# PathologyFoundation/plip

Measured on NVIDIA H100. Metric: image-text pairs/sec (224x224, 77-tok), higher is better.
Workload: dtype bf16

## Files before the change

### plip_b200/csrc/gemm_wgmma.cu

```cuda
#include "gemm.cuh"
#include "wgmma.cuh"

#include <stdio.h>
#include <stdlib.h>

namespace plip {

namespace {

constexpr int BM = 64;
constexpr int BK = 64;
constexpr int kThreads = 288;
constexpr int kConsumerWarps = 8;
constexpr uint32_t A_STAGE = BM * BK * 2;
constexpr uint32_t kStoreStageBytes = 16 * 128;

constexpr int x_boxes(int BN, int EPI) {
  return EPI != EPI_BIAS_RESID_F32 ? 2 : BN == 192 ? 3 : 2;
}

template <int BN, int EPI>
struct Cfg {
  static constexpr uint32_t B_STAGE = BN * BK * 2;
  static constexpr uint32_t STAGE = A_STAGE + B_STAGE;
  static constexpr int XBOXES = x_boxes(BN, EPI);
  static constexpr uint32_t EPI_BYTES = kConsumerWarps * XBOXES * kStoreStageBytes;
  static constexpr uint32_t BAR_BYTES = EPI == EPI_BIAS_RESID_F32 ? 512 : 256;
  static constexpr uint32_t ALIGN_SLACK = 1024;
  static constexpr int kMaxStages = (227 * 1024 - BAR_BYTES - EPI_BYTES - ALIGN_SLACK) / STAGE;
  static constexpr int STAGES = kMaxStages > 8 ? 8 : kMaxStages;
  static constexpr uint32_t SMEM_BYTES = STAGES * STAGE + EPI_BYTES + BAR_BYTES + ALIGN_SLACK;
};

struct GemmDev {
  int M, N, K;
  const float* bias;
  const float* rowscale;
  void* out;
  int ldo;
  const float* pos;
  int patches, seq;
  const float* colsum;
  const float2* stats_in;
  int n_partials;
  __nv_bfloat16* xb_out;
  float2* stats_out;
};

template <bool F16, int BN>
__device__ __forceinline__ void wgmma_ss(float (&d)[BN / 2], uint64_t adesc, uint64_t bdesc, uint32_t scale_d) {
  if constexpr (BN == 128) wgmma_ss_n128<F16>(d, adesc, bdesc, scale_d);
  else if constexpr (BN == 192) wgmma_ss_n192<F16>(d, adesc, bdesc, scale_d);
  else wgmma_ss_n256<F16>(d, adesc, bdesc, scale_d);
}

__device__ __forceinline__ float2 ln_row_terms(const GemmDev& p, int grow) {
  float s1 = 0.f, s2 = 0.f;
#pragma unroll
  for (int j = 0; j < kStatSlots; ++j) {
    const float2 t = (grow < p.M && j < p.n_partials) ? __ldg(p.stats_in + static_cast<size_t>(grow) * kStatSlots + j)
                                                      : make_float2(0.f, 0.f);
    s1 += t.x;
    s2 += t.y;
  }
  const float inv_k = 1.0f / static_cast<float>(p.K);
  const float mean = s1 * inv_k;
  const float rstd = rsqrtf(fmaxf(s2 * inv_k - mean * mean, 0.f) + kLnEps);
  return make_float2(-rstd * mean, rstd);
}

template <int BN, int EPI, bool F16>
__device__ __forceinline__ void epilogue_warp(const GemmDev& p, const CUtensorMap* tmC, float (&d)[BN / 2], uint32_t stage_smem,
                                              uint32_t& stage_sel, uint32_t xbar, int row_base, int col_base, int n_blk, int lane,
                                              float2 ln0, float2 ln1) {
  constexpr bool LN_FOLD = (EPI == EPI_LN_BIAS_BF16 || EPI == EPI_LN_BIAS_GELU_BF16);
  constexpr bool GELU = (EPI == EPI_BIAS_GELU_BF16 || EPI == EPI_LN_BIAS_GELU_BF16);
  constexpr bool HAS_BIAS = (EPI == EPI_BIAS_BF16 || EPI == EPI_BIAS_GELU_BF16 || EPI == EPI_BIAS_RESID_F32 || LN_FOLD);
  constexpr bool OUT_BF16 = (EPI == EPI_BIAS_BF16 || EPI == EPI_BIAS_GELU_BF16 || LN_FOLD);
  const int q = lane & 3, rr = lane >> 2;
  const int row0 = row_base + rr, row1 = row0 + 8;

  if constexpr (EPI == EPI_NULL) {
    float acc = 0.f;
#pragma unroll
    for (int i = 0; i < BN / 2; ++i) acc += d[i];
    if (acc == 1.2345e30f && p.M < 0) reinterpret_cast<float*>(p.out)[0] = acc;
  } else if constexpr (OUT_BF16) {
#pragma unroll
    for (int blk = 0; blk < BN / 64; ++blk) {
      const uint32_t buf = stage_smem + (stage_sel & 1u) * kStoreStageBytes;
      ++stage_sel;
      if (lane == 0) tma_store_wait_read_but_one();
      __syncwarp();
#pragma unroll
      for (int jj = 0; jj < 8; ++jj) {
        const int j = blk * 8 + jj;
        const int col = col_base + 8 * j + 2 * q;
        const float2 b = __ldg(reinterpret_cast<const float2*>(p.bias + col));
        float v00 = d[4 * j + 0], v01 = d[4 * j + 1], v10 = d[4 * j + 2], v11 = d[4 * j + 3];
        if constexpr (LN_FOLD) {
          const float2 cs = __ldg(reinterpret_cast<const float2*>(p.colsum + col));
          v00 = fmaf(ln0.y, v00, fmaf(ln0.x, cs.x, b.x));
          v01 = fmaf(ln0.y, v01, fmaf(ln0.x, cs.y, b.y));
          v10 = fmaf(ln1.y, v10, fmaf(ln1.x, cs.x, b.x));
          v11 = fmaf(ln1.y, v11, fmaf(ln1.x, cs.y, b.y));
        } else {
          v00 += b.x; v01 += b.y; v10 += b.x; v11 += b.y;
        }
        if constexpr (GELU) {
          v00 = quick_gelu(v00); v01 = quick_gelu(v01); v10 = quick_gelu(v10); v11 = quick_gelu(v11);
        }
        st_shared_b32(buf + rr * 128 + ((jj ^ rr) << 4) + q * 4, pack_op2<F16>(v00, v01));
        st_shared_b32(buf + (rr + 8) * 128 + ((jj ^ rr) << 4) + q * 4, pack_op2<F16>(v10, v11));
      }
      fence_proxy_async_smem();
      __syncwarp();
      if (lane == 0) {
        tma_store_2d(tmC, buf, col_base + blk * 64, row_base);
        tma_store_commit();
      }
    }
  } else if constexpr (EPI == EPI_BIAS_RESID_F32) {
    constexpr int kChunkCols = 32;
    constexpr int kChunks = BN / kChunkCols;
    constexpr int NB = x_boxes(BN, EPI);
    static_assert(kChunks % NB == 0, "every tile must start at staging block 0");
    constexpr int kUses = kChunks / NB;
    const bool ok0 = row0 < p.M, ok1 = row1 < p.M;
    const bool emit = p.xb_out != nullptr;
    const size_t o0 = static_cast<size_t>(ok0 ? row0 : 0) * p.ldo + col_base + 2 * q;
    const size_t o1 = o0 + 8 * static_cast<size_t>(p.ldo);
    uint32_t ph0 = 0;
    if constexpr (kUses % 2 != 0) ph0 = stage_sel++ & 1u;
    auto fetch = [&](int c) {
      if (lane == 0) {
        const uint32_t bar = xbar + 8u * (c % NB);
        mbar_arrive_expect_tx(bar, kStoreStageBytes);
        tma_load_2d(stage_smem + (c % NB) * kStoreStageBytes, tmC, bar, 2 * (col_base + c * kChunkCols), row_base);
      }
    };
    if (lane == 0) tma_store_wait_read();
    __syncwarp();
#pragma unroll
    for (int c = 0; c < NB; ++c) fetch(c);
    float st[2][2] = {};
#pragma unroll
    for (int c = 0; c < kChunks; ++c) {
      const int h = c < kChunks / 2 ? 0 : 1;
      mbar_wait(xbar + 8u * (c % NB), ph0 ^ ((c / NB) & 1u));
      const uint32_t buf = stage_smem + (c % NB) * kStoreStageBytes;
#pragma unroll
      for (int jj = 0; jj < kChunkCols / 8; ++jj) {
        const int j = c * (kChunkCols / 8) + jj;
        const int col = col_base + 8 * j + 2 * q;
        const uint32_t xoff = (((2 * jj + (q >> 1)) ^ rr) << 4) + (q & 1) * 8;
        const float2 b = __ldg(reinterpret_cast<const float2*>(p.bias + col));
        const float2 v0 = make_float2(d[4 * j + 0] + b.x, d[4 * j + 1] + b.y);
        const float2 v1 = make_float2(d[4 * j + 2] + b.x, d[4 * j + 3] + b.y);
        if (ok0) {
          const float2 x = ld_shared_f32x2(buf + rr * 128 + xoff);
          const float2 y = make_float2(x.x + v0.x, x.y + v0.y);
          st_shared_f32x2(buf + rr * 128 + xoff, y);
          if (emit) {
            *reinterpret_cast<uint32_t*>(p.xb_out + o0 + 8 * j) = pack_op2<F16>(y.x, y.y);
            st[0][0] += y.x + y.y;
            st[0][1] = fmaf(y.x, y.x, fmaf(y.y, y.y, st[0][1]));
          }
        }
        if (ok1) {
          const float2 x = ld_shared_f32x2(buf + (rr + 8) * 128 + xoff);
          const float2 y = make_float2(x.x + v1.x, x.y + v1.y);
          st_shared_f32x2(buf + (rr + 8) * 128 + xoff, y);
          if (emit) {
            *reinterpret_cast<uint32_t*>(p.xb_out + o1 + 8 * j) = pack_op2<F16>(y.x, y.y);
            st[1][0] += y.x + y.y;
            st[1][1] = fmaf(y.x, y.x, fmaf(y.y, y.y, st[1][1]));
          }
        }
      }
      fence_proxy_async_smem();
      __syncwarp();
      if (lane == 0) {
        tma_store_2d(tmC, buf, 2 * (col_base + c * kChunkCols), row_base);
        tma_store_commit();
      }
      if (c + NB < kChunks) {
        if (lane == 0) tma_store_wait_read();
        fetch(c + NB);
      }
      if (emit && (c + 1) % (kChunks / 2) == 0) {
#pragma unroll
        for (int r = 0; r < 2; ++r) {
          float a = st[r][0], b = st[r][1];
#pragma unroll
          for (int o = 1; o < 4; o <<= 1) {
            a += __shfl_xor_sync(0xffffffffu, a, o);
            b += __shfl_xor_sync(0xffffffffu, b, o);
          }
          if (q == 0 && (r == 0 ? ok0 : ok1))
            p.stats_out[static_cast<size_t>(row0 + 8 * r) * kStatSlots + 2 * n_blk + h] = make_float2(a, b);
          st[r][0] = 0.f;
          st[r][1] = 0.f;
        }
      }
    }
  } else {
    float* out = reinterpret_cast<float*>(p.out);
    const bool ok0 = row0 < p.M, ok1 = row1 < p.M;
    float rs0 = 1.f, rs1 = 1.f;
    size_t o0 = static_cast<size_t>(ok0 ? row0 : 0) * p.ldo, o1 = static_cast<size_t>(ok1 ? row1 : 0) * p.ldo;
    if constexpr (EPI == EPI_SIM_F32) {
      rs0 = ok0 ? __ldg(p.rowscale + row0) : 0.f;
      rs1 = ok1 ? __ldg(p.rowscale + row1) : 0.f;
    }
    size_t q0 = 0, q1 = 0;
    if constexpr (EPI == EPI_PATCH_F32) {
      const int r0 = ok0 ? row0 : 0, r1 = ok1 ? row1 : 0;
      const int b0 = r0 / p.patches, b1 = r1 / p.patches;
      o0 = static_cast<size_t>(b0 * p.seq + 1 + (r0 - b0 * p.patches)) * p.ldo;
      o1 = static_cast<size_t>(b1 * p.seq + 1 + (r1 - b1 * p.patches)) * p.ldo;
      q0 = static_cast<size_t>(1 + (r0 - b0 * p.patches)) * p.N;
      q1 = static_cast<size_t>(1 + (r1 - b1 * p.patches)) * p.N;
    }
#pragma unroll
    for (int j = 0; j < BN / 8; ++j) {
      const int col = col_base + 8 * j + 2 * q;
      float2 v0 = make_float2(d[4 * j + 0], d[4 * j + 1]), v1 = make_float2(d[4 * j + 2], d[4 * j + 3]);
      if constexpr (HAS_BIAS) {
        const float2 b = __ldg(reinterpret_cast<const float2*>(p.bias + col));
        v0.x += b.x; v0.y += b.y; v1.x += b.x; v1.y += b.y;
      }
      if constexpr (EPI == EPI_SIM_F32) {
        const float2 cs = __ldg(reinterpret_cast<const float2*>(p.bias + col));
        if (ok0) *reinterpret_cast<float2*>(out + o0 + col) = make_float2(v0.x * rs0 * cs.x, v0.y * rs0 * cs.y);
        if (ok1) *reinterpret_cast<float2*>(out + o1 + col) = make_float2(v1.x * rs1 * cs.x, v1.y * rs1 * cs.y);
      } else if constexpr (EPI == EPI_PATCH_F32) {
        if (ok0) {
          const float2 e = __ldg(reinterpret_cast<const float2*>(p.pos + q0 + col));
          *reinterpret_cast<float2*>(out + o0 + col) = make_float2(v0.x + e.x, v0.y + e.y);
        }
        if (ok1) {
          const float2 e = __ldg(reinterpret_cast<const float2*>(p.pos + q1 + col));
          *reinterpret_cast<float2*>(out + o1 + col) = make_float2(v1.x + e.x, v1.y + e.y);
        }
      } else {
        if (ok0) *reinterpret_cast<float2*>(out + o0 + col) = v0;
        if (ok1) *reinterpret_cast<float2*>(out + o1 + col) = v1;
      }
    }
  }
}

template <int CG, int BN, int EPI, bool F16>
__global__ void __launch_bounds__(kThreads, 1)
gemm_kernel(const __grid_constant__ CUtensorMap tmA, const __grid_constant__ CUtensorMap tmB,
            const __grid_constant__ CUtensorMap tmC, const GemmDev p) {
  using C = Cfg<BN, EPI>;
  constexpr int STAGES = C::STAGES;
  extern __shared__ uint8_t smem_raw[];
  const uint32_t smem_base = (smem_u32(smem_raw) + 1023u) & ~1023u;
  const uint32_t epi_base = smem_base + STAGES * C::STAGE;
  const uint32_t bar_base = epi_base + C::EPI_BYTES;
  auto full_bar = [&](int s) { return bar_base + 8u * s; };
  auto empty_bar = [&](int s) { return bar_base + 8u * (STAGES + s); };
  const uint32_t resid_bar = bar_base + 8u * (2 * STAGES);
  static_assert(8 * (2 * STAGES + (EPI == EPI_BIAS_RESID_F32 ? C::XBOXES * kConsumerWarps : 0)) <= C::BAR_BYTES,
                "barrier area too small");

  const int warp = threadIdx.x >> 5;
  const int lane = threadIdx.x & 31;
  const int wg = warp >> 2;
  const uint32_t cta_rank = (CG > 1) ? cluster_ctarank() : 0u;

  if (threadIdx.x == 0) {
    tma_prefetch_desc(&tmA);
    tma_prefetch_desc(&tmB);
    for (int s = 0; s < STAGES; ++s) {
      mbar_init(full_bar(s), 1);
      mbar_init(empty_bar(s), CG);
    }
    if constexpr (EPI == EPI_BIAS_RESID_F32) {
      tma_prefetch_desc(&tmC);
      for (int i = 0; i < C::XBOXES * kConsumerWarps; ++i) mbar_init(resid_bar + 8u * i, 1);
    }
    fence_mbar_init();
  }
  if constexpr (CG > 1) cluster_sync_all(); else __syncthreads();

  const int num_n_blk = p.N / BN;
  const int num_m_blk = (p.M + BM * CG - 1) / (BM * CG);
  const int num_tiles = num_m_blk * num_n_blk;
  const int num_kb = p.K / BK;
  const int tile0 = blockIdx.x / CG;
  const int tile_step = gridDim.x / CG;
  const int my_tiles = (num_tiles - tile0 + tile_step - 1) / tile_step;

  if (wg == 2) {
    if (lane == 0) {
      int s = 0;
      uint32_t ph = 0;
      for (int t = tile0; t < num_tiles; t += tile_step) {
        const int m0 = ((t / num_n_blk) * CG + cta_rank) * BM;
        const int n0 = (t % num_n_blk) * BN;
        for (int kb = 0; kb < num_kb; ++kb) {
          mbar_wait(empty_bar(s), ph ^ 1u);
          const uint32_t sa = smem_base + s * C::STAGE;
          const uint32_t sb = sa + A_STAGE;
          mbar_arrive_expect_tx(full_bar(s), C::STAGE);
          tma_load_2d(sa, &tmA, full_bar(s), kb * BK, m0);
          if constexpr (CG == 1) {
            tma_load_2d(sb, &tmB, full_bar(s), kb * BK, n0);
          } else {
            tma_load_2d_mc(sb + cta_rank * (C::B_STAGE / 2), &tmB, full_bar(s), kb * BK, n0 + cta_rank * (BN / 2), 0x3);
          }
          if (++s == STAGES) { s = 0; ph ^= 1u; }
        }
      }
    }
    __syncwarp();
  } else {
    const int wtid = threadIdx.x & 127;
    auto release = [&](int s) {
      if (wtid == 0) mbar_arrive(empty_bar(s));
      if constexpr (CG > 1) {
        if (wtid == 32) mbar_arrive_cluster(mapa_shared(empty_bar(s), cta_rank ^ 1u));
      }
    };
    float d[BN / 2];
    int s = 0;
    uint32_t ph = 0;
    auto skip_tile = [&]() {
      s += num_kb;
      ph ^= static_cast<uint32_t>(s / STAGES) & 1u;
      s %= STAGES;
    };
    uint32_t stage_sel = 0;
    const uint32_t my_turn = 1u + wg, other_turn = 2u - wg;
    const int rounds = (my_tiles + 1) / 2;
    if (wg == 1) skip_tile();
    for (int r = 0; r < rounds; ++r) {
      const int i = 2 * r + wg;
      const int t = tile0 + i * tile_step;
      const int n_blk = t % num_n_blk;
      const int m0 = ((t / num_n_blk) * CG + cta_rank) * BM;
      const int wrow = m0 + (warp & 3) * 16;
      float2 ln0 = make_float2(0.f, 1.f), ln1 = make_float2(0.f, 1.f);
      if constexpr (EPI == EPI_LN_BIAS_BF16 || EPI == EPI_LN_BIAS_GELU_BF16) {
        if (i < my_tiles) {
          ln0 = ln_row_terms(p, wrow + (lane >> 2));
          ln1 = ln_row_terms(p, wrow + (lane >> 2) + 8);
        }
      }
      if (wg == 1 || r > 0) named_barrier_sync<256>(my_turn);
      if (i >= my_tiles) break;
      int prev = -1;
      for (int kb = 0; kb < num_kb; ++kb) {
        mbar_wait(full_bar(s), ph);
        const uint32_t sa = smem_base + s * C::STAGE;
        const uint64_t adesc = make_smem_desc_sw128(sa, 1024, 16);
        const uint64_t bdesc = make_smem_desc_sw128(sa + A_STAGE, 1024, 16);
        wgmma_pin(d);
        wgmma_fence();
#pragma unroll
        for (int k = 0; k < BK / 16; ++k) wgmma_ss<F16, BN>(d, adesc + 2 * k, bdesc + 2 * k, (kb | k) != 0 ? 1u : 0u);
        wgmma_commit();
        wgmma_wait<1>();
        if (prev >= 0) release(prev);
        prev = s;
        if (++s == STAGES) { s = 0; ph ^= 1u; }
      }
      if (wg == 0 || r + 1 < rounds) named_barrier_arrive<256>(other_turn);
      wgmma_wait<0>();
      wgmma_pin(d);
      release(prev);
      skip_tile();
      epilogue_warp<BN, EPI, F16>(p, &tmC, d, epi_base + warp * C::XBOXES * kStoreStageBytes, stage_sel,
                                  resid_bar + 8u * C::XBOXES * warp, wrow,
                                  n_blk * BN, n_blk, lane, ln0, ln1);
    }
    if (lane == 0) tma_store_wait_all();
    __syncwarp();
  }
  if constexpr (CG > 1) cluster_sync_all();
}

int env_int(const char* name, int dflt) {
  const char* v = getenv(name);
  return v ? atoi(v) : dflt;
}

template <int CG, int BN, int EPI, bool F16>
int launch_inst(const GemmArgs& g, cudaStream_t stream) {
  using C = Cfg<BN, EPI>;
  auto kern = gemm_kernel<CG, BN, EPI, F16>;
  static unsigned long long configured = 0;
  static int max_groups = 0;
  if (first_use_on_device(configured)) {
    PLIP_CUDA_CHECK(cudaFuncSetAttribute(kern, cudaFuncAttributeMaxDynamicSharedMemorySize, (int)C::SMEM_BYTES));
    int dev = 0, sms = 0;
    PLIP_CUDA_CHECK(cudaGetDevice(&dev));
    PLIP_CUDA_CHECK(cudaDeviceGetAttribute(&sms, cudaDevAttrMultiProcessorCount, dev));
    max_groups = sms / CG;
    if (CG >= 2) {
      cudaLaunchConfig_t q = {};
      q.gridDim = dim3(sms / CG * CG);
      q.blockDim = dim3(kThreads);
      q.dynamicSmemBytes = C::SMEM_BYTES;
      cudaLaunchAttribute qa[1];
      qa[0].id = cudaLaunchAttributeClusterDimension;
      qa[0].val.clusterDim.x = CG; qa[0].val.clusterDim.y = 1; qa[0].val.clusterDim.z = 1;
      q.attrs = qa; q.numAttrs = 1;
      int n_clusters = 0;
      PLIP_CUDA_CHECK(cudaOccupancyMaxActiveClusters(&n_clusters, kern, &q));
      if (n_clusters > 0 && n_clusters < max_groups) max_groups = n_clusters;
    }
    PLIP_REQUIRE(max_groups > 0, "launch_gemm: no resident CTA fits (cg=%d bn=%d)", CG, BN);
  }
  CUtensorMap tmA, tmB;
  if (int rc = make_tmap_bf16_2d(&tmA, g.A, g.M, g.K, (uint64_t)g.lda * 2, BM, BK)) return rc;
  if (int rc = make_tmap_bf16_2d(&tmB, g.W, g.N, g.K, (uint64_t)g.ldw * 2, BN / CG, BK)) return rc;
  constexpr bool kOutBf16 = (EPI == EPI_BIAS_BF16 || EPI == EPI_BIAS_GELU_BF16 || EPI == EPI_LN_BIAS_BF16 ||
                             EPI == EPI_LN_BIAS_GELU_BF16);
  CUtensorMap tmC = tmA;
  if (kOutBf16)
    if (int rc = make_tmap_bf16_2d(&tmC, g.out, g.M, g.N, (uint64_t)g.ldo * 2, 16, 64)) return rc;
  if (EPI == EPI_BIAS_RESID_F32)
    if (int rc = make_tmap_bf16_2d(&tmC, g.out, g.M, 2 * (uint64_t)g.N, (uint64_t)g.ldo * 4, 16, 64)) return rc;

  GemmDev p;
  p.M = g.M; p.N = g.N; p.K = g.K;
  p.bias = g.bias; p.rowscale = g.rowscale; p.out = g.out; p.ldo = g.ldo; p.pos = g.pos;
  p.patches = g.patches; p.seq = g.seq;
  p.colsum = g.colsum; p.stats_in = g.stats_in; p.n_partials = g.n_partials;
  p.xb_out = g.xb_out; p.stats_out = g.stats_out;
  if (g.n_tiles_used) *g.n_tiles_used = 2 * (g.N / BN);

  const int num_tiles = ((g.M + BM * CG - 1) / (BM * CG)) * (g.N / BN);
  const int groups = max_groups < num_tiles ? max_groups : num_tiles;
  PLIP_CUDA_CHECK(launch_kernel(kern, dim3(groups * CG), dim3(kThreads), C::SMEM_BYTES, stream, CG, tmA, tmB, tmC, p));
  return 0;
}

template <int CG, int BN, bool F16>
int launch_epi_fmt(const GemmArgs& g, cudaStream_t stream) {
  switch (g.epi) {
    case EPI_BIAS_BF16: return launch_inst<CG, BN, EPI_BIAS_BF16, F16>(g, stream);
    case EPI_BIAS_GELU_BF16: return launch_inst<CG, BN, EPI_BIAS_GELU_BF16, F16>(g, stream);
    case EPI_BIAS_RESID_F32: return launch_inst<CG, BN, EPI_BIAS_RESID_F32, F16>(g, stream);
    case EPI_PATCH_F32: return launch_inst<CG, BN, EPI_PATCH_F32, F16>(g, stream);
    case EPI_F32: return launch_inst<CG, BN, EPI_F32, F16>(g, stream);
    case EPI_LN_BIAS_BF16: return launch_inst<CG, BN, EPI_LN_BIAS_BF16, F16>(g, stream);
    case EPI_LN_BIAS_GELU_BF16: return launch_inst<CG, BN, EPI_LN_BIAS_GELU_BF16, F16>(g, stream);
    case EPI_NULL: return launch_inst<CG, BN, EPI_NULL, F16>(g, stream);
    case EPI_SIM_F32: return launch_inst<CG, BN, EPI_SIM_F32, F16>(g, stream);
    default: set_last_error("launch_gemm: bad epilogue %d", g.epi); return -2;
  }
}
template <int CG, int BN>
int launch_epi(const GemmArgs& g, cudaStream_t stream) {
  return g.f16 ? launch_epi_fmt<CG, BN, true>(g, stream) : launch_epi_fmt<CG, BN, false>(g, stream);
}

}

int launch_gemm(const GemmArgs& g, cudaStream_t stream) {
  PLIP_REQUIRE(g.M > 0 && g.N > 0 && g.K > 0, "launch_gemm: empty problem M=%d N=%d K=%d", g.M, g.N, g.K);
  PLIP_REQUIRE(g.K % BK == 0, "launch_gemm: K=%d must be a multiple of %d", g.K, BK);
  PLIP_REQUIRE(g.N % 128 == 0 || g.N % 192 == 0, "launch_gemm: N=%d must be a multiple of 128 or 192", g.N);
  PLIP_REQUIRE((g.lda % 8) == 0 && (g.ldw % 8) == 0 && (g.ldo % 8) == 0,
               "launch_gemm: leading dimensions must be multiples of 8 elements");
  PLIP_REQUIRE((reinterpret_cast<uintptr_t>(g.A) & 15) == 0 && (reinterpret_cast<uintptr_t>(g.W) & 15) == 0 &&
               (reinterpret_cast<uintptr_t>(g.out) & 15) == 0,
               "launch_gemm: operands must be 16-byte aligned");
  if (g.epi == EPI_LN_BIAS_BF16 || g.epi == EPI_LN_BIAS_GELU_BF16)
    PLIP_REQUIRE(g.colsum && g.stats_in && g.bias && g.n_partials >= 1 && g.n_partials <= kStatSlots,
                 "launch_gemm: LayerNorm-folded epilogue needs colsum, stats and 1..%d partials", kStatSlots);
  if (g.epi == EPI_SIM_F32)
    PLIP_REQUIRE(g.bias && g.rowscale, "launch_gemm: the similarity epilogue needs row and column scales");
  if (g.epi == EPI_PATCH_F32)
    PLIP_REQUIRE(g.patches >= 1 && g.seq == g.patches + 1, "launch_gemm: patch epilogue with %d patches, %d rows",
                 g.patches, g.seq);
  if (g.xb_out || g.stats_out)
    PLIP_REQUIRE(g.epi == EPI_BIAS_RESID_F32 && g.xb_out && g.stats_out,
                 "launch_gemm: xb/stats outputs belong to the residual epilogue");
  static const int env_cg = env_int("PLIP_GEMM_CG", 0);
  static const int env_bn = env_int("PLIP_GEMM_BN", 0);
  int cg = g.force_cg ? g.force_cg : (env_cg ? env_cg : 2);
  int bn = g.force_bn ? g.force_bn : (env_bn ? env_bn : 256);
  if (g.N % bn != 0) bn = 128;
  if (!g.force_bn && g.stats_out && 2 * (g.N / bn) > kStatSlots && g.N % 256 == 0) bn = 256;
  PLIP_REQUIRE((cg == 1 || cg == 2) && (bn == 128 || bn == 256 || (bn == 192 && cg == 2)),
               "launch_gemm: bad config cg=%d bn=%d", cg, bn);
  PLIP_REQUIRE(!g.stats_out || 2 * (g.N / bn) <= kStatSlots, "launch_gemm: N=%d / BN=%d exceeds %d statistics slots",
               g.N, bn, kStatSlots);
  if (cg == 1) return bn == 256 ? launch_epi<1, 256>(g, stream) : launch_epi<1, 128>(g, stream);
  if (bn == 192) return launch_epi<2, 192>(g, stream);
  return bn == 256 ? launch_epi<2, 256>(g, stream) : launch_epi<2, 128>(g, stream);
}

}
```

Measured before the change: 26640.

## Add warp-specialized streaming residual GEMM with separate MMA and epilogue warpgroups

Result: no change. 26760, median of 6 (+0.5%).

```diff
diff --git a/plip_b200/csrc/gemm_wgmma.cu b/plip_b200/csrc/gemm_wgmma.cu
--- a/plip_b200/csrc/gemm_wgmma.cu
+++ b/plip_b200/csrc/gemm_wgmma.cu
@@ -3,6 +3,8 @@
 
 #include <stdio.h>
 #include <stdlib.h>
+
+#include <type_traits>
 
 namespace plip {
 
@@ -30,6 +32,23 @@
   static constexpr int kMaxStages = (227 * 1024 - BAR_BYTES - EPI_BYTES - ALIGN_SLACK) / STAGE;
   static constexpr int STAGES = kMaxStages > 8 ? 8 : kMaxStages;
   static constexpr uint32_t SMEM_BYTES = STAGES * STAGE + EPI_BYTES + BAR_BYTES + ALIGN_SLACK;
+};
+
+struct StreamCfg {
+  static constexpr int BN = 128;
+  static constexpr int kThreads = 13 * 32;
+  static constexpr uint32_t B_STAGE = BN * BK * 2;
+  static constexpr uint32_t STAGE = A_STAGE + B_STAGE;
+  static constexpr int XBOXES = 4;
+  static constexpr int ACC_BUFS = 2;
+  static constexpr uint32_t ACC_BYTES = BM * BN * 4;
+  static constexpr uint32_t EPI_BYTES = 8 * XBOXES * kStoreStageBytes;
+  static constexpr uint32_t BAR_BYTES = 512;
+  static constexpr uint32_t ALIGN_SLACK = 1024;
+  static constexpr int kMaxStages =
+      (227 * 1024 - BAR_BYTES - EPI_BYTES - ACC_BUFS * ACC_BYTES - ALIGN_SLACK) / STAGE;
+  static constexpr int STAGES = kMaxStages > 8 ? 8 : kMaxStages;
+  static constexpr uint32_t SMEM_BYTES = STAGES * STAGE + ACC_BUFS * ACC_BYTES + EPI_BYTES + BAR_BYTES + ALIGN_SLACK;
 };
 
 struct GemmDev {
@@ -384,15 +403,241 @@
   if constexpr (CG > 1) cluster_sync_all();
 }
 
+__device__ __forceinline__ void st_shared_f32x4(uint32_t addr, float a, float b, float c, float d) {
+  asm volatile("st.shared.v4.f32 [%0], {%1, %2, %3, %4};" ::"r"(addr), "f"(a), "f"(b), "f"(c), "f"(d) : "memory");
+}
+__device__ __forceinline__ float4 ld_shared_f32x4(uint32_t addr) {
+  float4 v;
+  asm volatile("ld.shared.v4.f32 {%0, %1, %2, %3}, [%4];" : "=f"(v.x), "=f"(v.y), "=f"(v.z), "=f"(v.w) : "r"(addr)
+               : "memory");
+  return v;
+}
+
+template <bool F16>
+__global__ void __launch_bounds__(StreamCfg::kThreads, 1)
+gemm_resid_stream_kernel(const __grid_constant__ CUtensorMap tmA, const __grid_constant__ CUtensorMap tmB,
+                         const __grid_constant__ CUtensorMap tmC, const GemmDev p) {
+  constexpr int CG = 2;
+  using C = StreamCfg;
+  constexpr int BN = C::BN;
+  constexpr int STAGES = C::STAGES;
+  constexpr int NB = C::XBOXES;
+  constexpr int kChunkCols = 32;
+  constexpr int kChunks = BN / kChunkCols;
+  extern __shared__ uint8_t smem_raw[];
+  const uint32_t smem_base = (smem_u32(smem_raw) + 1023u) & ~1023u;
+  const uint32_t acc_base = smem_base + STAGES * C::STAGE;
+  const uint32_t box_base = acc_base + C::ACC_BUFS * C::ACC_BYTES;
+  const uint32_t bar_base = box_base + C::EPI_BYTES;
+  auto full_bar = [&](int s) { return bar_base + 8u * s; };
+  auto empty_bar = [&](int s) { return bar_base + 8u * (STAGES + s); };
+  auto acc_full = [&](int b) { return bar_base + 8u * (2 * STAGES + b); };
+  auto acc_empty = [&](int b) { return bar_base + 8u * (2 * STAGES + 2 + b); };
+  const uint32_t box_bar = bar_base + 8u * (2 * STAGES + 4);
+  static_assert(C::ACC_BUFS == 2, "one accumulator buffer per epilogue warpgroup");
+  static_assert(8 * (2 * STAGES + 4 + 8 * NB) <= C::BAR_BYTES, "barrier area too small");
+
+  const int warp = threadIdx.x >> 5;
+  const int lane = threadIdx.x & 31;
+  const int wg = warp >> 2;
+  const uint32_t cta_rank = cluster_ctarank();
+
+  if (threadIdx.x == 0) {
+    tma_prefetch_desc(&tmA);
+    tma_prefetch_desc(&tmB);
+    tma_prefetch_desc(&tmC);
+    for (int s = 0; s < STAGES; ++s) {
+      mbar_init(full_bar(s), 1);
+      mbar_init(empty_bar(s), CG);
+    }
+    for (int b = 0; b < 2; ++b) {
+      mbar_init(acc_full(b), 128);
+      mbar_init(acc_empty(b), 128);
+    }
+    for (int i = 0; i < 8 * NB; ++i) mbar_init(box_bar + 8u * i, 1);
+    fence_mbar_init();
+  }
+  cluster_sync_all();
+
+  const int num_n_blk = p.N / BN;
+  const int num_m_blk = (p.M + BM * CG - 1) / (BM * CG);
+  const int num_tiles = num_m_blk * num_n_blk;
+  const int num_kb = p.K / BK;
+  const int tile0 = blockIdx.x / CG;
+  const int tile_step = gridDim.x / CG;
+  const int my_tiles = (num_tiles - tile0 + tile_step - 1) / tile_step;
+
+  if (wg == 3) {
+    if (lane == 0) {
+      int s = 0;
+      uint32_t ph = 0;
+      for (int t = tile0; t < num_tiles; t += tile_step) {
+        const int m0 = ((t / num_n_blk) * CG + cta_rank) * BM;
+        const int n0 = (t % num_n_blk) * BN;
+        for (int kb = 0; kb < num_kb; ++kb) {
+          mbar_wait(empty_bar(s), ph ^ 1u);
+          const uint32_t sa = smem_base + s * C::STAGE;
+          const uint32_t sb = sa + A_STAGE;
+          mbar_arrive_expect_tx(full_bar(s), C::STAGE);
+          tma_load_2d(sa, &tmA, full_bar(s), kb * BK, m0);
+          tma_load_2d_mc(sb + cta_rank * (C::B_STAGE / 2), &tmB, full_bar(s), kb * BK, n0 + cta_rank * (BN / 2), 0x3);
+          if (++s == STAGES) { s = 0; ph ^= 1u; }
+        }
+      }
+    }
+    __syncwarp();
+  } else if (wg == 0) {
+    const int wtid = threadIdx.x;
+    auto release = [&](int s) {
+      if (wtid == 0) mbar_arrive(empty_bar(s));
+      if (wtid == 32) mbar_arrive_cluster(mapa_shared(empty_bar(s), cta_rank ^ 1u));
+    };
+    float d[BN / 2];
+    int s = 0;
+    uint32_t ph = 0;
+    for (int i = 0; i < my_tiles; ++i) {
+      int prev = -1;
+      for (int kb = 0; kb < num_kb; ++kb) {
+        mbar_wait(full_bar(s), ph);
+        const uint32_t sa = smem_base + s * C::STAGE;
+        const uint64_t adesc = make_smem_desc_sw128(sa, 1024, 16);
+        const uint64_t bdesc = make_smem_desc_sw128(sa + A_STAGE, 1024, 16);
+        wgmma_pin(d);
+        wgmma_fence();
+#pragma unroll
+        for (int k = 0; k < BK / 16; ++k) wgmma_ss<F16, BN>(d, adesc + 2 * k, bdesc + 2 * k, (kb | k) != 0 ? 1u : 0u);
+        wgmma_commit();
+        wgmma_wait<1>();
+        if (prev >= 0) release(prev);
+        prev = s;
+        if (++s == STAGES) { s = 0; ph ^= 1u; }
+      }
+      wgmma_wait<0>();
+      wgmma_pin(d);
+      release(prev);
+      const int b = i & 1;
+      mbar_wait(acc_empty(b), ((i >> 1) & 1u) ^ 1u);
+      const uint32_t dst = acc_base + b * C::ACC_BYTES + (warp * (BN / 8) * 32 + lane) * 16;
+#pragma unroll
+      for (int j = 0; j < BN / 8; ++j) st_shared_f32x4(dst + j * 512, d[4 * j], d[4 * j + 1], d[4 * j + 2], d[4 * j + 3]);
+      mbar_arrive(acc_full(b));
+    }
+  } else {
+    const int e = wg - 1;
+    const int ew = warp & 3;
+    const int ewarp = warp - 4;
+    const uint32_t boxes = box_base + ewarp * NB * kStoreStageBytes;
+    const uint32_t xbar = box_bar + 8u * NB * ewarp;
+    const int n_mine = (my_tiles - e + 1) / 2;
+    const int total = n_mine * kChunks;
+    auto tile_of = [&](int li) { return tile0 + (e + 2 * li) * tile_step; };
+    auto fetch = [&](int c) {
+      if (lane == 0) {
+        const int t = tile_of(c / kChunks);
+        const int col = (t % num_n_blk) * BN + (c % kChunks) * kChunkCols;
+        const int row = ((t / num_n_blk) * CG + cta_rank) * BM + ew * 16;
+        const uint32_t bar = xbar + 8u * (c % NB);
+        mbar_arrive_expect_tx(bar, kStoreStageBytes);
+        tma_load_2d(boxes + (c % NB) * kStoreStageBytes, &tmC, bar, 2 * col, row);
+      }
+    };
+    for (int c = 0; c < NB && c < total; ++c) fetch(c);
+    const int q = lane & 3, rr = lane >> 2;
+    const bool emit = p.xb_out != nullptr;
+    for (int li = 0; li < n_mine; ++li) {
+      const int t = tile_of(li);
+      const int n_blk = t % num_n_blk;
+      const int col_base = n_blk * BN;
+      const int row_base = ((t / num_n_blk) * CG + cta_rank) * BM + ew * 16;
+      const int row0 = row_base + rr, row1 = row0 + 8;
+      const bool ok0 = row0 < p.M, ok1 = row1 < p.M;
+      const size_t o0 = static_cast<size_t>(ok0 ? row0 : 0) * p.ldo + col_base + 2 * q;
+      const size_t o1 = o0 + 8 * static_cast<size_t>(p.ldo);
+      mbar_wait(acc_full(e), li & 1u);
+      const uint32_t src = acc_base + e * C::ACC_BYTES + (ew * (BN / 8) * 32 + lane) * 16;
+      float st[2][2] = {};
+#pragma unroll
+      for (int cc = 0; cc < kChunks; ++cc) {
+        const int c = li * kChunks + cc;
+        mbar_wait(xbar + 8u * (c % NB), (c / NB) & 1u);
+        const uint32_t buf = boxes + (c % NB) * kStoreStageBytes;
+#pragma unroll
+        for (int jj = 0; jj < kChunkCols / 8; ++jj) {
+          const int j = cc * (kChunkCols / 8) + jj;
+          const int col = col_base + 8 * j + 2 * q;
+          const uint32_t xoff = (((2 * jj + (q >> 1)) ^ rr) << 4) + (q & 1) * 8;
+          const float4 a = ld_shared_f32x4(src + j * 512);
+          const float2 bb = __ldg(reinterpret_cast<const float2*>(p.bias + col));
+          const float2 v0 = make_float2(a.x + bb.x, a.y + bb.y);
+          const float2 v1 = make_float2(a.z + bb.x, a.w + bb.y);
+          if (ok0) {
+            const float2 x = ld_shared_f32x2(buf + rr * 128 + xoff);
+            const float2 y = make_float2(x.x + v0.x, x.y + v0.y);
+            st_shared_f32x2(buf + rr * 128 + xoff, y);
+            if (emit) {
+              *reinterpret_cast<uint32_t*>(p.xb_out + o0 + 8 * j) = pack_op2<F16>(y.x, y.y);
+              st[0][0] += y.x + y.y;
+              st[0][1] = fmaf(y.x, y.x, fmaf(y.y, y.y, st[0][1]));
+            }
+          }
+          if (ok1) {
+            const float2 x = ld_shared_f32x2(buf + (rr + 8) * 128 + xoff);
+            const float2 y = make_float2(x.x + v1.x, x.y + v1.y);
+            st_shared_f32x2(buf + (rr + 8) * 128 + xoff, y);
+            if (emit) {
+              *reinterpret_cast<uint32_t*>(p.xb_out + o1 + 8 * j) = pack_op2<F16>(y.x, y.y);
+              st[1][0] += y.x + y.y;
+              st[1][1] = fmaf(y.x, y.x, fmaf(y.y, y.y, st[1][1]));
+            }
+          }
+        }
+        if (cc == kChunks - 1) mbar_arrive(acc_empty(e));
+        fence_proxy_async_smem();
+        __syncwarp();
+        if (lane == 0) {
+          tma_store_2d(&tmC, buf, 2 * (col_base + cc * kChunkCols), row_base);
+          tma_store_commit();
+        }
+        if (c >= 1 && c - 1 + NB < total) {
+          if (lane == 0) tma_store_wait_read_but_one();
+          fetch(c - 1 + NB);
+        }
+      }
+      if (emit) {
+#pragma unroll
+        for (int r = 0; r < 2; ++r) {
+          float sa = st[r][0], sb = st[r][1];
+#pragma unroll
+          for (int o = 1; o < 4; o <<= 1) {
+            sa += __shfl_xor_sync(0xffffffffu, sa, o);
+            sb += __shfl_xor_sync(0xffffffffu, sb, o);
+          }
+          if (q == 0 && (r == 0 ? ok0 : ok1))
+            p.stats_out[static_cast<size_t>(row0 + 8 * r) * kStatSlots + n_blk] = make_float2(sa, sb);
+        }
+      }
+    }
+    if (lane == 0) tma_store_wait_all();
+    __syncwarp();
+  }
+  cluster_sync_all();
+}
+
 int env_int(const char* name, int dflt) {
   const char* v = getenv(name);
   return v ? atoi(v) : dflt;
 }
 
-template <int CG, int BN, int EPI, bool F16>
+template <int CG, int BN, int EPI, bool F16, bool STREAM = false>
 int launch_inst(const GemmArgs& g, cudaStream_t stream) {
-  using C = Cfg<BN, EPI>;
-  auto kern = gemm_kernel<CG, BN, EPI, F16>;
+  static_assert(!STREAM || (CG == 2 && EPI == EPI_BIAS_RESID_F32), "the streaming body is the CG 2 residual GEMM");
+  static_assert(!STREAM || BN == StreamCfg::BN, "the streaming body runs 128-column tiles");
+  using C = std::conditional_t<STREAM, StreamCfg, Cfg<BN, EPI>>;
+  constexpr int threads = STREAM ? StreamCfg::kThreads : kThreads;
+  auto kern = [] {
+    if constexpr (STREAM) return gemm_resid_stream_kernel<F16>;
+    else return gemm_kernel<CG, BN, EPI, F16>;
+  }();
   static unsigned long long configured = 0;
   static int max_groups = 0;
   if (first_use_on_device(configured)) {
@@ -404,7 +649,7 @@
     if (CG >= 2) {
       cudaLaunchConfig_t q = {};
       q.gridDim = dim3(sms / CG * CG);
-      q.blockDim = dim3(kThreads);
+      q.blockDim = dim3(threads);
       q.dynamicSmemBytes = C::SMEM_BYTES;
       cudaLaunchAttribute qa[1];
       qa[0].id = cudaLaunchAttributeClusterDimension;
@@ -433,11 +678,11 @@
   p.patches = g.patches; p.seq = g.seq;
   p.colsum = g.colsum; p.stats_in = g.stats_in; p.n_partials = g.n_partials;
   p.xb_out = g.xb_out; p.stats_out = g.stats_out;
-  if (g.n_tiles_used) *g.n_tiles_used = 2 * (g.N / BN);
+  if (g.n_tiles_used) *g.n_tiles_used = STREAM ? g.N / 128 : 2 * (g.N / BN);
 
   const int num_tiles = ((g.M + BM * CG - 1) / (BM * CG)) * (g.N / BN);
   const int groups = max_groups < num_tiles ? max_groups : num_tiles;
-  PLIP_CUDA_CHECK(launch_kernel(kern, dim3(groups * CG), dim3(kThreads), C::SMEM_BYTES, stream, CG, tmA, tmB, tmC, p));
+  PLIP_CUDA_CHECK(launch_kernel(kern, dim3(groups * CG), dim3(threads), C::SMEM_BYTES, stream, CG, tmA, tmB, tmC, p));
   return 0;
 }
 
@@ -459,6 +704,10 @@
 template <int CG, int BN>
 int launch_epi(const GemmArgs& g, cudaStream_t stream) {
   return g.f16 ? launch_epi_fmt<CG, BN, true>(g, stream) : launch_epi_fmt<CG, BN, false>(g, stream);
+}
+int launch_stream(const GemmArgs& g, cudaStream_t stream) {
+  return g.f16 ? launch_inst<2, StreamCfg::BN, EPI_BIAS_RESID_F32, true, true>(g, stream)
+               : launch_inst<2, StreamCfg::BN, EPI_BIAS_RESID_F32, false, true>(g, stream);
 }
 
 }
@@ -483,9 +732,20 @@
   if (g.xb_out || g.stats_out)
     PLIP_REQUIRE(g.epi == EPI_BIAS_RESID_F32 && g.xb_out && g.stats_out,
                  "launch_gemm: xb/stats outputs belong to the residual epilogue");
+  const bool route_only = g.force_cg == -1;
+  if (g.force_bn == -StreamCfg::BN) {
+    PLIP_REQUIRE(g.epi == EPI_BIAS_RESID_F32 && (g.force_cg == 0 || g.force_cg == 2 || route_only) &&
+                 g.N % StreamCfg::BN == 0,
+                 "launch_gemm: the streaming body runs the residual epilogue with cg 2 and N a multiple of %d "
+                 "(epi=%d cg=%d N=%d)", StreamCfg::BN, g.epi, g.force_cg, g.N);
+    PLIP_REQUIRE(!g.stats_out || g.N / 128 <= kStatSlots, "launch_gemm: N=%d exceeds %d statistics slots", g.N,
+                 kStatSlots);
+    if (route_only) return 2;
+    return launch_stream(g, stream);
+  }
   static const int env_cg = env_int("PLIP_GEMM_CG", 0);
   static const int env_bn = env_int("PLIP_GEMM_BN", 0);
-  int cg = g.force_cg ? g.force_cg : (env_cg ? env_cg : 2);
+  int cg = g.force_cg > 0 ? g.force_cg : (env_cg ? env_cg : 2);
   int bn = g.force_bn ? g.force_bn : (env_bn ? env_bn : 256);
   if (g.N % bn != 0) bn = 128;
   if (!g.force_bn && g.stats_out && 2 * (g.N / bn) > kStatSlots && g.N % 256 == 0) bn = 256;
@@ -493,6 +753,9 @@
                "launch_gemm: bad config cg=%d bn=%d", cg, bn);
   PLIP_REQUIRE(!g.stats_out || 2 * (g.N / bn) <= kStatSlots, "launch_gemm: N=%d / BN=%d exceeds %d statistics slots",
                g.N, bn, kStatSlots);
+  const bool stream_body = !g.force_bn && g.epi == EPI_BIAS_RESID_F32 && g.K <= g.N && cg == 2 && bn == 256;
+  if (route_only) return stream_body ? 2 : 1;
+  if (stream_body) return launch_stream(g, stream);
   if (cg == 1) return bn == 256 ? launch_epi<1, 256>(g, stream) : launch_epi<1, 128>(g, stream);
   if (bn == 192) return launch_epi<2, 192>(g, stream);
   return bn == 256 ? launch_epi<2, 256>(g, stream) : launch_epi<2, 128>(g, stream);
```

## Add 4-CTA cluster GEMM with weight-tile multicast and heuristic selection

Applied to the files above, without the earlier changes.

Result: no change. 27000 before, 26990 after, median of 6 (-0.1%).

```diff
diff --git a/plip_b200/csrc/gemm_wgmma.cu b/plip_b200/csrc/gemm_wgmma.cu
--- a/plip_b200/csrc/gemm_wgmma.cu
+++ b/plip_b200/csrc/gemm_wgmma.cu
@@ -255,6 +255,7 @@
 __global__ void __launch_bounds__(kThreads, 1)
 gemm_kernel(const __grid_constant__ CUtensorMap tmA, const __grid_constant__ CUtensorMap tmB,
             const __grid_constant__ CUtensorMap tmC, const GemmDev p) {
+  static_assert(CG == 1 || CG == 2 || CG == 4, "clusters of 1, 2 or 4 CTAs");
   using C = Cfg<BN, EPI>;
   constexpr int STAGES = C::STAGES;
   extern __shared__ uint8_t smem_raw[];
@@ -311,7 +312,8 @@
           if constexpr (CG == 1) {
             tma_load_2d(sb, &tmB, full_bar(s), kb * BK, n0);
           } else {
-            tma_load_2d_mc(sb + cta_rank * (C::B_STAGE / 2), &tmB, full_bar(s), kb * BK, n0 + cta_rank * (BN / 2), 0x3);
+            tma_load_2d_mc(sb + cta_rank * (C::B_STAGE / CG), &tmB, full_bar(s), kb * BK, n0 + cta_rank * (BN / CG),
+                           (1u << CG) - 1u);
           }
           if (++s == STAGES) { s = 0; ph ^= 1u; }
         }
@@ -324,6 +326,10 @@
       if (wtid == 0) mbar_arrive(empty_bar(s));
       if constexpr (CG > 1) {
         if (wtid == 32) mbar_arrive_cluster(mapa_shared(empty_bar(s), cta_rank ^ 1u));
+      }
+      if constexpr (CG > 2) {
+        if (wtid == 64) mbar_arrive_cluster(mapa_shared(empty_bar(s), cta_rank ^ 2u));
+        if (wtid == 96) mbar_arrive_cluster(mapa_shared(empty_bar(s), cta_rank ^ 3u));
       }
     };
     float d[BN / 2];
@@ -390,7 +396,7 @@
 }
 
 template <int CG, int BN, int EPI, bool F16>
-int launch_inst(const GemmArgs& g, cudaStream_t stream) {
+int resident_groups() {
   using C = Cfg<BN, EPI>;
   auto kern = gemm_kernel<CG, BN, EPI, F16>;
   static unsigned long long configured = 0;
@@ -414,7 +420,20 @@
       PLIP_CUDA_CHECK(cudaOccupancyMaxActiveClusters(&n_clusters, kern, &q));
       if (n_clusters > 0 && n_clusters < max_groups) max_groups = n_clusters;
     }
-    PLIP_REQUIRE(max_groups > 0, "launch_gemm: no resident CTA fits (cg=%d bn=%d)", CG, BN);
+  }
+  PLIP_REQUIRE(max_groups > 0, "launch_gemm: no resident CTA fits (cg=%d bn=%d)", CG, BN);
+  return max_groups;
+}
+
+template <int CG, int BN, int EPI, bool F16>
+int launch_inst(const GemmArgs& g, cudaStream_t stream, int* resident) {
+  using C = Cfg<BN, EPI>;
+  auto kern = gemm_kernel<CG, BN, EPI, F16>;
+  const int max_groups = resident_groups<CG, BN, EPI, F16>();
+  if (max_groups < 0) return max_groups;
+  if (resident) {
+    *resident = max_groups;
+    return 0;
   }
   CUtensorMap tmA, tmB;
   if (int rc = make_tmap_bf16_2d(&tmA, g.A, g.M, g.K, (uint64_t)g.lda * 2, BM, BK)) return rc;
@@ -442,24 +461,39 @@
 }
 
 template <int CG, int BN, bool F16>
-int launch_epi_fmt(const GemmArgs& g, cudaStream_t stream) {
+int launch_epi_fmt(const GemmArgs& g, cudaStream_t stream, int* resident) {
   switch (g.epi) {
-    case EPI_BIAS_BF16: return launch_inst<CG, BN, EPI_BIAS_BF16, F16>(g, stream);
-    case EPI_BIAS_GELU_BF16: return launch_inst<CG, BN, EPI_BIAS_GELU_BF16, F16>(g, stream);
-    case EPI_BIAS_RESID_F32: return launch_inst<CG, BN, EPI_BIAS_RESID_F32, F16>(g, stream);
-    case EPI_PATCH_F32: return launch_inst<CG, BN, EPI_PATCH_F32, F16>(g, stream);
-    case EPI_F32: return launch_inst<CG, BN, EPI_F32, F16>(g, stream);
-    case EPI_LN_BIAS_BF16: return launch_inst<CG, BN, EPI_LN_BIAS_BF16, F16>(g, stream);
-    case EPI_LN_BIAS_GELU_BF16: return launch_inst<CG, BN, EPI_LN_BIAS_GELU_BF16, F16>(g, stream);
-    case EPI_NULL: return launch_inst<CG, BN, EPI_NULL, F16>(g, stream);
-    case EPI_SIM_F32: return launch_inst<CG, BN, EPI_SIM_F32, F16>(g, stream);
+    case EPI_BIAS_BF16: return launch_inst<CG, BN, EPI_BIAS_BF16, F16>(g, stream, resident);
+    case EPI_BIAS_GELU_BF16: return launch_inst<CG, BN, EPI_BIAS_GELU_BF16, F16>(g, stream, resident);
+    case EPI_BIAS_RESID_F32: return launch_inst<CG, BN, EPI_BIAS_RESID_F32, F16>(g, stream, resident);
+    case EPI_PATCH_F32: return launch_inst<CG, BN, EPI_PATCH_F32, F16>(g, stream, resident);
+    case EPI_F32: return launch_inst<CG, BN, EPI_F32, F16>(g, stream, resident);
+    case EPI_LN_BIAS_BF16: return launch_inst<CG, BN, EPI_LN_BIAS_BF16, F16>(g, stream, resident);
+    case EPI_LN_BIAS_GELU_BF16: return launch_inst<CG, BN, EPI_LN_BIAS_GELU_BF16, F16>(g, stream, resident);
+    case EPI_NULL: return launch_inst<CG, BN, EPI_NULL, F16>(g, stream, resident);
+    case EPI_SIM_F32: return launch_inst<CG, BN, EPI_SIM_F32, F16>(g, stream, resident);
     default: set_last_error("launch_gemm: bad epilogue %d", g.epi); return -2;
   }
 }
 template <int CG, int BN>
-int launch_epi(const GemmArgs& g, cudaStream_t stream) {
-  return g.f16 ? launch_epi_fmt<CG, BN, true>(g, stream) : launch_epi_fmt<CG, BN, false>(g, stream);
-}
+int launch_epi(const GemmArgs& g, cudaStream_t stream, int* resident) {
+  return g.f16 ? launch_epi_fmt<CG, BN, true>(g, stream, resident) : launch_epi_fmt<CG, BN, false>(g, stream, resident);
+}
+
+int dispatch(const GemmArgs& g, cudaStream_t stream, int cg, int bn, int* resident) {
+  PLIP_REQUIRE((cg == 1 || cg == 2 || cg == 4) && (bn == 128 || bn == 256 || (bn == 192 && cg == 2)),
+               "launch_gemm: bad config cg=%d bn=%d", cg, bn);
+  if (cg == 1) return bn == 256 ? launch_epi<1, 256>(g, stream, resident) : launch_epi<1, 128>(g, stream, resident);
+  if (cg == 4) return bn == 256 ? launch_epi<4, 256>(g, stream, resident) : launch_epi<4, 128>(g, stream, resident);
+  if (bn == 192) return launch_epi<2, 192>(g, stream, resident);
+  return bn == 256 ? launch_epi<2, 256>(g, stream, resident) : launch_epi<2, 128>(g, stream, resident);
+}
+
+bool cg4_pays(const GemmArgs& g) {
+  const bool short_16bit = (g.epi == EPI_BIAS_BF16 || g.epi == EPI_LN_BIAS_BF16) && g.K >= 768;
+  return short_16bit || g.epi == EPI_PATCH_F32;
+}
+constexpr int kCg4MinWaves = 4;
 
 }
 
@@ -485,17 +519,22 @@
                  "launch_gemm: xb/stats outputs belong to the residual epilogue");
   static const int env_cg = env_int("PLIP_GEMM_CG", 0);
   static const int env_bn = env_int("PLIP_GEMM_BN", 0);
-  int cg = g.force_cg ? g.force_cg : (env_cg ? env_cg : 2);
+  int cg = g.force_cg ? g.force_cg : env_cg;
   int bn = g.force_bn ? g.force_bn : (env_bn ? env_bn : 256);
   if (g.N % bn != 0) bn = 128;
   if (!g.force_bn && g.stats_out && 2 * (g.N / bn) > kStatSlots && g.N % 256 == 0) bn = 256;
-  PLIP_REQUIRE((cg == 1 || cg == 2) && (bn == 128 || bn == 256 || (bn == 192 && cg == 2)),
-               "launch_gemm: bad config cg=%d bn=%d", cg, bn);
   PLIP_REQUIRE(!g.stats_out || 2 * (g.N / bn) <= kStatSlots, "launch_gemm: N=%d / BN=%d exceeds %d statistics slots",
                g.N, bn, kStatSlots);
-  if (cg == 1) return bn == 256 ? launch_epi<1, 256>(g, stream) : launch_epi<1, 128>(g, stream);
-  if (bn == 192) return launch_epi<2, 192>(g, stream);
-  return bn == 256 ? launch_epi<2, 256>(g, stream) : launch_epi<2, 128>(g, stream);
-}
-
-}
+  if (cg == 0) {
+    cg = 2;
+    if (bn != 192 && cg4_pays(g)) {
+      int resident4 = 0;
+      if (int rc = dispatch(g, stream, 4, bn, &resident4)) return rc;
+      const long long tiles4 = static_cast<long long>((g.M + 4 * BM - 1) / (4 * BM)) * (g.N / bn);
+      if (tiles4 >= static_cast<long long>(kCg4MinWaves) * resident4) cg = 4;
+    }
+  }
+  return dispatch(g, stream, cg, bn, nullptr);
+}
+
+}
```
